# leabouffaut/DAS4Whales

Hardware: AMD Instinct MI355X
Metric: channel-samples/sec through f-k filter + matched-filter (higher is better)
Workload: dtype f32 (matched filter: 2 x f16 split operands on the matrix cores, f32 accumulate); 1 GPU; 20000 channels x 120000 samples float32 per GPU, classic f-k fan mask (fk_filter_design defaults), stages fk+mf, HF+LF fin-call templates; api=public, parallelism=independent channel blocks x1

## Files before the change

### das4whales_amd/csrc/xcorr_mm.hip

```cpp
#include <cstdlib>

#include "mm_common.h"

namespace d4w {

constexpr int kMmCH = 4096;
constexpr int kMmCHPair = 8192;
constexpr int kMmGroup = 4096;
constexpr int kMmKS = 6;
constexpr int kMmKSLong = 8;
constexpr int kMmKSMax = 16;
constexpr int kMmSection = 32 * kMmKSMax - 16;
constexpr int kMmMaxSupport = 32 * kMmKSLong - 15;
constexpr int kMmMaxSections = 16;
constexpr int kMmThreads = 256;
template <int KSM, int CH = kMmCH>
struct MmGeom {
    static constexpr int G = CH > kMmGroup ? CH / kMmGroup : 1;
    static constexpr int GL = CH / G;
    static constexpr int Halo = 32 * KSM;
    static constexpr int Stage = CH + Halo;
    static constexpr int Q = (Stage + 4 * kMmThreads - 1) / (4 * kMmThreads);
    static constexpr int LastQ = (Stage - (Q - 1) * 4 * kMmThreads) / 4;
    static constexpr int GStage = GL + Halo;
    static constexpr int Arr = G * GStage + 8;
    static constexpr int QG = GL / (4 * kMmThreads);
    static constexpr int Blk = CH / 4;
    static constexpr int Pb = G == 1 ? Blk : Blk / 4;
    static constexpr size_t lds_bytes(bool tail) {
        return (size_t)4 * Arr * sizeof(mm_half) + 8 * G * sizeof(float) + (tail ? ((size_t)2 * Pb + 2 * 16 * G) * sizeof(float) : 0);
    }
    static_assert(CH % (4 * kMmThreads) == 0 && GL % (4 * kMmThreads) == 0 && Halo <= 4 * kMmThreads, "a group is whole loads; its halo lies in one");
};

struct MmArgs {
    const float* x;
    const float* xnext;
    const double* mean;
    const float* maxabs;
    const float* taps;
    float* y0;
    float* y1;
    int nx, ns, ld_next, n_next, ltaps, len0, len1;
    float* rowmax0;
    float* rowmax1;
    int clamp;
    int shift;
    int accumulate;
    float tail0, tail1;
};

__device__ __forceinline__ int mm_tile(int wv, int ti) { return wv + 4 * ti; }

__device__ __forceinline__ float mm_wave_scan(float v) {
#ifdef D4W_EMU
    const int lane = (int)(threadIdx.x & 63);
    for (int off = 1; off < 64; off <<= 1) {
        const float n = __shfl_up(v, (unsigned)off);
        if (lane >= off) v += n;
    }
    return v;
#else
    auto dpp = [](float x, auto ctrl, auto rmask) {
        return __int_as_float(__builtin_amdgcn_update_dpp(0, __float_as_int(x), decltype(ctrl)::value, decltype(rmask)::value, 0xf, false));
    };
    v += dpp(v, std::integral_constant<int, 0x111>{}, std::integral_constant<int, 0xf>{});
    v += dpp(v, std::integral_constant<int, 0x112>{}, std::integral_constant<int, 0xf>{});
    v += dpp(v, std::integral_constant<int, 0x114>{}, std::integral_constant<int, 0xf>{});
    v += dpp(v, std::integral_constant<int, 0x118>{}, std::integral_constant<int, 0xf>{});
    v += dpp(v, std::integral_constant<int, 0x142>{}, std::integral_constant<int, 0xa>{});
    v += dpp(v, std::integral_constant<int, 0x143>{}, std::integral_constant<int, 0xc>{});
    return v;
#endif
}

template <int KS0, int KS1, int WPS, bool TAIL = false, bool WMAX = false, int CH = kMmCH>
__global__ __launch_bounds__(kMmThreads, WPS) void xcorr_mm_rows(MmArgs P) {
    constexpr int KSM = KS0 > KS1 ? KS0 : KS1;
    using GEO = MmGeom<KSM, CH>;
    constexpr int kMmHalo = GEO::Halo, kMmStage = GEO::Stage, kMmQ = GEO::Q, kMmLastQ = GEO::LastQ, kMmArr = GEO::Arr;
    constexpr int G = GEO::G, GL = GEO::GL, QG = GEO::QG, kPb = GEO::Pb;
    D4W_DYN_LDS(smem_raw);
    mm_half* lds = reinterpret_cast<mm_half*>(smem_raw);
    float* red = reinterpret_cast<float*>(lds + 4 * kMmArr);
    float* pb = red + 8 * G;
    float* wt = pb + 2 * kPb;
    const int tid = (int)threadIdx.x;
    const int lane = tid & 63, wv = mm_uniform(tid >> 6);
    const int n16 = lane & 15, g = lane >> 4;
    const int ns = P.ns;

    mm_h8 a0h[KS0], a0l[KS0];
    mm_h8 a1h[KS1 ? KS1 : 1], a1l[KS1 ? KS1 : 1];
    float osc0 = 1.f, osc1 = 1.f;
    constexpr bool kRows = TAIL;
    const int nchunk = (ns + CH - 1) / CH;
    int row_n = 0, cin_n = 0;
    size_t roff_n = 0;
    bool more_n = false;
    int left_n = 0, d_row = 0, d_cin = 0;
    if constexpr (kRows) {
        row_n = (int)blockIdx.x;
        more_n = row_n < P.nx;
    } else {
        const long long total = (long long)P.nx * nchunk;
        const int nparts = min(8, (int)gridDim.x);
        const int xcd = (int)blockIdx.x % nparts, wq = (int)blockIdx.x / nparts, nq = ((int)gridDim.x - xcd + nparts - 1) / nparts;
        const long long lo_c = total * xcd / nparts, hi_c = total * (xcd + 1) / nparts;
        const long long c_first = lo_c + wq;
        left_n = c_first < hi_c ? (int)((hi_c - c_first + nq - 1) / nq) : 0;
        row_n = (int)(c_first / nchunk);
        cin_n = (int)(c_first - (long long)row_n * nchunk);
        d_row = nq / nchunk;
        d_cin = nq - d_row * nchunk;
        more_n = left_n > 0;
    }
    roff_n = (size_t)row_n * ns;
    const size_t d_off = (size_t)(kRows ? (int)gridDim.x : d_row) * ns;
    auto advance = [&]() {
        if constexpr (kRows) {
            if (++cin_n == nchunk) { cin_n = 0; row_n += (int)gridDim.x; roff_n += d_off; }
            more_n = row_n < P.nx;
        } else {
            cin_n += d_cin; row_n += d_row; roff_n += d_off;
            if (cin_n >= nchunk) { cin_n -= nchunk; ++row_n; roff_n += (size_t)ns; }
            more_n = --left_n > 0;
        }
    };
    {
        float* tl = reinterpret_cast<float*>(smem_raw);
        constexpr int TLP = 16 + kMmHalo;
        for (int i = tid; i < 2 * TLP; i += kMmThreads) {
            const int t = i / TLP, u = i - t * TLP - 15;
            const int L = t ? P.len1 : P.len0;
            float tv = (u >= 0 && u < L && (t == 0 || KS1 > 0)) ? P.taps[(size_t)t * P.ltaps + u] : 0.f;
            if constexpr (TAIL) {
                if (u < L && (t == 0 || KS1 > 0)) tv += t ? P.tail1 : P.tail0;
            }
            tl[i] = tv;
        }
        __syncthreads();
        auto build = [&](const float* tp, int L, auto& ah, auto& al, auto ks, float& osc) {
            constexpr int KS = decltype(ks)::value;
            float m = 0.f;
            for (int i = lane; i < TLP; i += 64) m = fmaxf(m, fabsf(tp[i]));
            for (int o = 32; o > 0; o >>= 1) m = fmaxf(m, __shfl_xor(m, o));
            float up, down;
            mm_pow2_scale(m, up, down);
            osc = up;
            (void)L;
            static_for<KS>([&](auto kq) {
                constexpr int kk = decltype(kq)::value;
                static_for<8>([&](auto jq) {
                    constexpr int j = decltype(jq)::value;
                    const float v = tp[15 + 32 * kk + 8 * g + j - n16] * down;
                    mm_half hi, lo;
                    mm_split(v, hi, lo);
                    mm_set(ah[kk], j, hi);
                    mm_set(al[kk], j, lo);
                });
            });
        };
        build(tl, P.len0, a0h, a0l, std::integral_constant<int, KS0>{}, osc0);
        if constexpr (KS1 > 0) build(tl + TLP, P.len1, a1h, a1l, std::integral_constant<int, KS1>{}, osc1);
        __syncthreads();
    }

    float4 pre[kMmQ];
    Mean2 mu_n{0.f, 0.f};
    float g_n = 1.f;
    bool heavy_n = false;
    bool tail_n = false;
    int c0_n = 0;

    auto issue = [&]() {
        c0_n = cin_n * CH;
        if (!kRows || cin_n == 0) {
            mu_n = mean2_load(P.mean, row_n);
            g_n = 1.f;
            if (P.maxabs) {
                const float a = P.maxabs[row_n];
                g_n = (a > 0.f) ? 1.0f / a : 0.f;
                heavy_n = fabsf(mu_n.hi) > 0.9921875f * a;
            }
        }
        const int s0 = c0_n + P.shift;
        tail_n = s0 + kMmStage > ns;
        const float* xr = P.x + roff_n;
        const bool al = (reinterpret_cast<uintptr_t>(xr + s0) & 15) == 0;
        if (al && s0 + kMmStage <= ns) {
            const float4* p = reinterpret_cast<const float4*>(xr + s0) + tid;
            static_for<kMmQ>([&](auto qq) {
                constexpr int q = decltype(qq)::value;
                if (q < kMmQ - 1 || tid < kMmLastQ) pre[q] = mm_load4_stream(p + q * kMmThreads);
            });
        } else {
            if (al && (ns & 3) == 0) {
                static_for<kMmQ>([&](auto qq) {
                    constexpr int q = decltype(qq)::value;
                    if (q < kMmQ - 1 || tid < kMmLastQ) {
                        const int i = s0 + 4 * (tid + q * kMmThreads);
                        const float4 v = *reinterpret_cast<const float4*>(xr + min(i, ns - 4));
                        pre[q] = (i < ns) ? v : make_float4(mu_n.hi, mu_n.hi, mu_n.hi, mu_n.hi);
                    }
                });
            } else {
                static_for<kMmQ>([&](auto qq) {
                    constexpr int q = decltype(qq)::value;
                    if (q < kMmQ - 1 || tid < kMmLastQ) {
                        const int i = s0 + 4 * (tid + q * kMmThreads);
                        const float a0 = xr[min(i, ns - 1)], a1 = xr[min(i + 1, ns - 1)], a2 = xr[min(i + 2, ns - 1)], a3 = xr[min(i + 3, ns - 1)];
                        pre[q] = make_float4(i < ns ? a0 : mu_n.hi, i + 1 < ns ? a1 : mu_n.hi, i + 2 < ns ? a2 : mu_n.hi, i + 3 < ns ? a3 : mu_n.hi);
                    }
                });
            }
            if (P.xnext && P.n_next > 0 && s0 + kMmStage > ns) {
                const float* xn = P.xnext + (size_t)row_n * P.ld_next;
                const int n_next = P.n_next;
                static_for<kMmQ>([&](auto qq) {
                    constexpr int q = decltype(qq)::value;
                    if (q < kMmQ - 1 || tid < kMmLastQ) {
                        const int d = s0 + 4 * (tid + q * kMmThreads) - ns;
                        const float b0 = xn[min(max(d, 0), n_next - 1)], b1 = xn[min(max(d + 1, 0), n_next - 1)];
                        const float b2 = xn[min(max(d + 2, 0), n_next - 1)], b3 = xn[min(max(d + 3, 0), n_next - 1)];
                        if (d >= 0 && d < n_next) pre[q].x = b0;
                        if (d + 1 >= 0 && d + 1 < n_next) pre[q].y = b1;
                        if (d + 2 >= 0 && d + 2 < n_next) pre[q].z = b2;
                        if (d + 3 >= 0 && d + 3 < n_next) pre[q].w = b3;
                    }
                });
            }
        }
    };

    if (more_n) issue();
    int buf = 0;
    float pst_hi = 0.f, pst_lo = 0.f;
    for (bool more = more_n; more; more = more_n) {
        const int row = row_n, c0 = c0_n, cin = cin_n;
        const size_t roff = roff_n;
        const Mean2 mu = mu_n;
        const bool tail = tail_n;
        const int n_valid = ns + ((P.xnext && P.n_next > 0) ? P.n_next : 0) - c0 - P.shift;
        const float gout = g_n;
        const bool own_scale = !P.maxabs || heavy_n;
        float gsc[G], osx[G];
        static_for<G>([&](auto gg) { gsc[decltype(gg)::value] = g_n; osx[decltype(gg)::value] = 1.f; });
        mm_half* bh = lds + (size_t)buf * 2 * kMmArr;
        mm_half* bl = bh + kMmArr;
        advance();
        if (TAIL && cin == 0) { pst_hi = 0.f; pst_lo = 0.f; }
        if (own_scale) {
            float m[G];
            static_for<G>([&](auto gg) { m[decltype(gg)::value] = 0.f; });
            static_for<kMmQ>([&](auto qq) {
                constexpr int q = decltype(qq)::value, gq = q / QG < G ? q / QG : G - 1;
                if (q < kMmQ - 1 || tid < kMmLastQ) {
                    const float4 v = pre[q];
                    const int at = 4 * (tid + q * kMmThreads);
                    float d0 = demean(v.x, mu), d1 = demean(v.y, mu), d2 = demean(v.z, mu), d3 = demean(v.w, mu);
                    if (tail) {
                        if (at >= n_valid) d0 = 0.f;
                        if (at + 1 >= n_valid) d1 = 0.f;
                        if (at + 2 >= n_valid) d2 = 0.f;
                        if (at + 3 >= n_valid) d3 = 0.f;
                    }
                    m[gq] = fmaxf(fmaxf(m[gq], fmaxf(fabsf(d0), fabsf(d1))), fmaxf(fabsf(d2), fabsf(d3)));
                    if constexpr (q >= QG && q < G * QG && q % QG == 0) {
                        if (tid < kMmHalo / 4) m[gq - 1] = fmaxf(fmaxf(m[gq - 1], fmaxf(fabsf(d0), fabsf(d1))), fmaxf(fabsf(d2), fabsf(d3)));
                    }
                }
            });
            static_for<G>([&](auto gg) {
                constexpr int gi = decltype(gg)::value;
                for (int o = 32; o > 0; o >>= 1) m[gi] = fmaxf(m[gi], __shfl_xor(m[gi], o));
                if (lane == 0) red[wv + 4 * (gi + G * buf)] = m[gi];
            });
            lds_barrier();
            static_for<G>([&](auto gg) {
                constexpr int gi = decltype(gg)::value;
                const float* r4 = red + 4 * (gi + G * buf);
                float up, down;
                mm_pow2_scale(fmaxf(fmaxf(r4[0], r4[1]), fmaxf(r4[2], r4[3])), up, down);
                osx[gi] = mm_uniform(up);
                gsc[gi] = mm_uniform(down);
            });
        }
        auto scaled = [&](const float4 v, int at, auto gg, float (&s)[4]) {
            constexpr int gi = decltype(gg)::value;
            const float mlg = -mu.lo * gsc[gi];
            s[0] = fmaf(v.x - mu.hi, gsc[gi], mlg); s[1] = fmaf(v.y - mu.hi, gsc[gi], mlg); s[2] = fmaf(v.z - mu.hi, gsc[gi], mlg); s[3] = fmaf(v.w - mu.hi, gsc[gi], mlg);
            if (P.clamp && !own_scale) static_for<4>([&](auto ee) { constexpr int e = decltype(ee)::value; s[e] = mm_clamp_half(s[e]); });
            if (tail) {
                static_for<4>([&](auto ee) { constexpr int e = decltype(ee)::value; if (at + e >= n_valid) s[e] = 0.f; });
            }
        };
        static_for<kMmQ>([&](auto qq) {
            constexpr int q = decltype(qq)::value, gq = q / QG < G ? q / QG : G - 1;
            float s[4] = {0.f, 0.f, 0.f, 0.f};
            const bool mine = q < kMmQ - 1 || tid < kMmLastQ;
            const int at = 4 * (tid + q * kMmThreads);
#ifdef D4W_MM_V_NOCONV
            if (mine && pre[q].x == 1.2345e30f) {
#else
            if (mine) {
#endif
                scaled(pre[q], at, std::integral_constant<int, gq>{}, s);
                mm_split_put4(s, bh + (at + gq * kMmHalo), bl + (at + gq * kMmHalo));
                if constexpr (q >= QG && q < G * QG && q % QG == 0) {
                    if (tid < kMmHalo / 4) {
                        float h4[4];
                        scaled(pre[q], at, std::integral_constant<int, gq - 1>{}, h4);
                        mm_split_put4(h4, bh + (at + (gq - 1) * kMmHalo), bl + (at + (gq - 1) * kMmHalo));
                    }
                }
            }
            if constexpr (TAIL && q < G * QG) {
                const float t4 = (s[0] + s[1]) + (s[2] + s[3]);
                const float inc = mm_wave_scan(t4);
                if constexpr (G == 1) pb[buf * kPb + kMmThreads * q + tid] = inc - t4;
                else if ((lane & 3) == 0) pb[buf * kPb + (kMmThreads / 4) * q + (tid >> 2)] = inc - t4;
                if (lane == 63) wt[buf * 16 * G + 4 * q + wv] = inc;
            }
        });
        if (more_n) issue();
        lds_barrier();
        float* ya = P.y0 + roff;
        float* yb = KS1 ? P.y1 + roff : nullptr;
        const bool valign = ((reinterpret_cast<uintptr_t>(ya + c0) & 15) == 0) && (!KS1 || (reinterpret_cast<uintptr_t>(yb + c0) & 15) == 0);
        float oxs[G], o0[G], o1[G];
        static_for<G>([&](auto gg) {
            constexpr int gi = decltype(gg)::value;
            oxs[gi] = (own_scale && P.maxabs) ? osx[gi] * gout : osx[gi];
            o0[gi] = osc0 * oxs[gi];
            o1[gi] = osc1 * oxs[gi];
        });
        float segoff[G], pstg[G];
        static_for<G>([&](auto gg) { segoff[decltype(gg)::value] = 0.f; pstg[decltype(gg)::value] = 0.f; });
        constexpr int NTW = CH / 256 / 4, NST = NTW * KSM, PF = 2;
        constexpr int TG = GL / 256;
        auto frag = [&](const mm_half* arr, int ti, int kk) -> mm_h8 {
            const int T = mm_tile(wv, ti);
            const int gr = 32 * T + 2 * n16 + g + 4 * kk;
            return *reinterpret_cast<const mm_h8*>(arr + (8 * gr + (4 * ti / TG) * kMmHalo));
        };
        mm_h8 fh[PF + 1], fl[PF + 1];
        static_for<PF>([&](auto ss) {
            constexpr int s_ = decltype(ss)::value;
            fh[s_] = frag(bh, s_ / KSM, s_ % KSM);
            fl[s_] = frag(bl, s_ / KSM, s_ % KSM);
        });
        mm_f4 c0h = mm_zero(), c0l = mm_zero(), c1h = mm_zero(), c1l = mm_zero();
        float vmax0 = -INFINITY, vmax1 = -INFINITY;
        float vsum = 0.f;
        static_for<NST>([&](auto ss) {
            constexpr int s_ = decltype(ss)::value, ti = s_ / KSM, kk = s_ % KSM;
            if constexpr (s_ + PF < NST) {
                fh[(s_ + PF) % (PF + 1)] = frag(bh, (s_ + PF) / KSM, (s_ + PF) % KSM);
                fl[(s_ + PF) % (PF + 1)] = frag(bl, (s_ + PF) / KSM, (s_ + PF) % KSM);
            }
            mm_sched_fence();
            const mm_h8 xh = fh[s_ % (PF + 1)], xl = fl[s_ % (PF + 1)];
#ifndef D4W_MM_V_NOMFMA
            if constexpr (kk < KS0) {
                c0h = mm_mfma(a0h[kk], xh, c0h);
                c0l = mm_mfma(a0h[kk], xl, c0l);
            }
            if constexpr (kk < KS1) {
                c1h = mm_mfma(a1h[kk], xh, c1h);
                c1l = mm_mfma(a1h[kk], xl, c1l);
            }
            if constexpr (kk < KS0) c0l = mm_mfma(a0l[kk], xh, c0l);
            if constexpr (kk < KS1) c1l = mm_mfma(a1l[kk], xh, c1l);
#else
            c0h[0] += (float)xh[0]; c0l[0] += (float)xl[0];
#endif
            mm_sched_fence();
            if constexpr (kk == KSM - 1) {
                constexpr int tg = 4 * ti / TG;
                const int T = mm_tile(wv, ti);
                const int kl = 256 * T + 16 * n16 + 4 * g;
                const int k = c0 + kl;
                if constexpr (ti == 0) {
                    if constexpr (TAIL) {
                        static_for<G>([&](auto gg) {
                            constexpr int gi = decltype(gg)::value;
                            const float w = lane < 16 ? wt[buf * 16 * G + 16 * gi + lane] : 0.f;
                            const float inc = mm_wave_scan(w);
                            segoff[gi] = inc - w;
                            pstg[gi] = pst_hi;
#ifdef D4W_EMU
                            const float own = __shfl(inc, 15);
#else
                            const float own = __builtin_bit_cast(float, __builtin_amdgcn_readlane(__builtin_bit_cast(int, inc), 15));
#endif
                            const double pd = ((double)pst_hi + (double)pst_lo) + (double)(own * oxs[gi]);
                            const float ph = (float)pd, pl2 = (float)(pd - (double)ph);
#ifdef D4W_EMU
                            pst_hi = ph; pst_lo = pl2;
#else
                            pst_hi = __builtin_bit_cast(float, __builtin_amdgcn_readfirstlane(__builtin_bit_cast(int, ph)));
                            pst_lo = __builtin_bit_cast(float, __builtin_amdgcn_readfirstlane(__builtin_bit_cast(int, pl2)));
#endif
                        });
                    }
                }
                float r0[4], r1[4];
                float a0 = 0.f, a1 = 0.f;
                if constexpr (TAIL) {
#ifdef D4W_EMU
                    const float so = __shfl(segoff[tg], T - tg * TG);
#else
                    const float so = __builtin_bit_cast(float, __builtin_amdgcn_readlane(__builtin_bit_cast(int, segoff[tg]), T - tg * TG));
#endif
                    const int pi = G == 1 ? kMmThreads * (T >> 2) + 64 * (T & 3) + 4 * n16 : (kMmThreads / 4) * (T >> 2) + 16 * (T & 3) + n16;
                    const float pbk = fmaf(so + pb[buf * kPb + pi], oxs[tg], pstg[tg]);
                    a0 = P.tail0 * pbk;
                    a1 = P.tail1 * pbk;
                }
                static_for<4>([&](auto rr) {
                    constexpr int r = decltype(rr)::value;
                    r0[r] = fmaf(fmaf(mm_get(c0l, r), kMmLoInv, mm_get(c0h, r)), o0[tg], a0);
                    if constexpr (KS1 > 0) r1[r] = fmaf(fmaf(mm_get(c1l, r), kMmLoInv, mm_get(c1h, r)), o1[tg], a1);
                });
                c0h = mm_zero(); c0l = mm_zero(); c1h = mm_zero(); c1l = mm_zero();
#ifdef D4W_MM_V_NOSTORE
                if (r0[0] != 1.2345e30f) { }
                else
#endif
                if (valign && k + 3 < ns) {
                    if (KS1 == 0 && P.accumulate) {
                        const float4 o = mm_load4_stream(reinterpret_cast<const float4*>(ya + k));
                        r0[0] += o.x; r0[1] += o.y; r0[2] += o.z; r0[3] += o.w;
                    }
                    mm_store4(ya + k, r0[0], r0[1], r0[2], r0[3]);
                    if constexpr (KS1 > 0) mm_store4(yb + k, r1[0], r1[1], r1[2], r1[3]);
                    if (WMAX) {
                        vmax0 = fmaxf(vmax0, fmaxf(fmaxf(r0[0], r0[1]), fmaxf(r0[2], r0[3])));
                        vsum += (r0[0] + r0[1]) + (r0[2] + r0[3]);
                        if constexpr (KS1 > 0) {
                            vmax1 = fmaxf(vmax1, fmaxf(fmaxf(r1[0], r1[1]), fmaxf(r1[2], r1[3])));
                            vsum += (r1[0] + r1[1]) + (r1[2] + r1[3]);
                        }
                    }
                } else {
                    for (int r = 0; r < 4; ++r)
                        if (k + r < ns) {
                            const float v0 = (KS1 == 0 && P.accumulate) ? ya[k + r] + r0[r] : r0[r];
                            ya[k + r] = v0;
                            if constexpr (KS1 > 0) yb[k + r] = r1[r];
                            if (WMAX) {
                                vmax0 = fmaxf(vmax0, v0);
                                vsum += v0;
                                if constexpr (KS1 > 0) { vmax1 = fmaxf(vmax1, r1[r]); vsum += r1[r]; }
                            }
                        }
                }
            }
        });
        if (WMAX) {
            for (int o = 32; o > 0; o >>= 1) {
                vmax0 = fmaxf(vmax0, __shfl_xor(vmax0, o));
                if constexpr (KS1 > 0) vmax1 = fmaxf(vmax1, __shfl_xor(vmax1, o));
            }
            const bool bad = __any(vsum != vsum);
            if (lane == 0) {
                mm_atomic_fmax(P.rowmax0 + row, bad ? __uint_as_float(0x7FC00000u) : vmax0);
                if constexpr (KS1 > 0) mm_atomic_fmax(P.rowmax1 + row, bad ? __uint_as_float(0x7FC00000u) : vmax1);
            }
        }
        buf ^= 1;
    }
}

}

using namespace d4w;


constexpr int mm_wps(int ks0, int ks1, bool tail, bool wmax) { return (ks1 == 0 && ks0 <= kMmKS && !(tail && wmax)) ? 3 : 2; }

template <int KS0, int KS1, bool TAIL, bool WMAX, int CH>
static int mm_launch_as(const MmArgs& Q, int grid, void* stream) {
    constexpr size_t lds = MmGeom<(KS0 > KS1 ? KS0 : KS1), CH>::lds_bytes(TAIL);
    void (*kern)(MmArgs) = xcorr_mm_rows<KS0, KS1, mm_wps(KS0, KS1, TAIL, WMAX), TAIL, WMAX, CH>;
    if (lds > 64 * 1024) D4W_HIP(hipFuncSetAttribute((const void*)kern, hipFuncAttributeMaxDynamicSharedMemorySize, (int)lds));
    D4W_LAUNCH(kern, dim3(grid), dim3(kMmThreads), lds, stream, Q);
    return D4W_OK;
}

template <int KS0, int KS1, bool TAIL, int CH = kMmCH>
static int mm_launch(const MmArgs& Q, int grid, void* stream) {
    return Q.rowmax0 ? mm_launch_as<KS0, KS1, TAIL, true, CH>(Q, grid, stream) : mm_launch_as<KS0, KS1, TAIL, false, CH>(Q, grid, stream);
}

template <bool TAIL>
static int mm_one_section(const MmArgs& Q, int grid, void* stream) {
    const int ks = ceil_div(Q.len0 + 15, 32);
    if (ks <= kMmKS) return mm_launch<kMmKS, 0, TAIL>(Q, grid, stream);
    if (ks <= kMmKSLong) return mm_launch<kMmKSLong, 0, TAIL>(Q, grid, stream);
    if (ks <= 12) return mm_launch<12, 0, TAIL>(Q, grid, stream);
    return mm_launch<kMmKSMax, 0, TAIL>(Q, grid, stream);
}

template <bool TAIL>
static int mm_pair(const MmArgs& P, int grid, void* stream) {
    if (ceil_div(P.len0 + 15, 32) <= 5) return mm_launch<5, kMmKS, TAIL, kMmCHPair>(P, grid, stream);
    return mm_launch<kMmKS, kMmKS, TAIL, kMmCHPair>(P, grid, stream);
}

static int mm_one_template(MmArgs Q, const float* taps, int len, bool tails, float tail, float* y, float* rowmax, int grid, void* stream) {
    const int nsec = (len <= 32 * kMmKSMax - 15) ? 1 : ceil_div(len, kMmSection);
    const int per = (nsec == 1) ? len : 16 * ceil_div(ceil_div(len, nsec), 16);
    Q.y0 = y;
    Q.y1 = nullptr;
    Q.rowmax1 = nullptr;
    Q.tail0 = tail;
    Q.tail1 = 0.f;
    for (int j = 0; j < nsec; ++j) {
        const int first = j * per;
        Q.taps = taps + first;
        Q.len0 = Q.len1 = std::min(per, len - first);
        Q.shift = first;
        Q.accumulate = j > 0;
        Q.rowmax0 = (j == nsec - 1) ? rowmax : nullptr;
        const int rc = tails ? mm_one_section<true>(Q, grid, stream) : mm_one_section<false>(Q, grid, stream);
        if (rc != D4W_OK) return rc;
    }
    return D4W_OK;
}

extern "C" {

int d4w_xcorr_mm_max_support(void) { return kMmSection * kMmMaxSections; }

int d4w_xcorr_mm_f32(const float* x, int nx, int ns, const float* xnext, int ld_next, int n_next, const double* mean,
                     const float* maxabs, const float* taps, int ntpl, int ltaps, int len0, int len1, float* y0, float* y1,
                     void* stream) {
    return d4w_xcorr_mm_rowmax_f32(x, nx, ns, xnext, ld_next, n_next, mean, maxabs, taps, ntpl, ltaps, len0, len1, y0, y1, nullptr,
                                   nullptr, stream);
}

int d4w_xcorr_mm_rowmax_f32(const float* x, int nx, int ns, const float* xnext, int ld_next, int n_next, const double* mean,
                            const float* maxabs, const float* taps, int ntpl, int ltaps, int len0, int len1, float* y0, float* y1,
                            float* rowmax0, float* rowmax1, void* stream) {
    return d4w_xcorr_mm_tail_f32(x, nx, ns, xnext, ld_next, n_next, mean, maxabs, taps, ntpl, ltaps, len0, len1, 0.0, 0.0, y0, y1,
                                 rowmax0, rowmax1, stream);
}

int d4w_xcorr_mm_tail_max_support(void) { return 32 * kMmKSMax - 15; }

int d4w_xcorr_mm_tail_f32(const float* x, int nx, int ns, const float* xnext, int ld_next, int n_next, const double* mean,
                          const float* maxabs, const float* taps, int ntpl, int ltaps, int len0, int len1, double tail0, double tail1,
                          float* y0, float* y1, float* rowmax0, float* rowmax1, void* stream) {
    if (!x || !y0 || !taps || nx < 1 || ns < 1) return fail(D4W_EINVAL, "bad argument");
    if (ntpl == 2 && ((rowmax0 == nullptr) != (rowmax1 == nullptr))) return fail(D4W_EINVAL, "rowmax0 and rowmax1 go together");
    if (ntpl < 1 || ntpl > 2 || (ntpl == 2 && !y1)) return fail(D4W_EINVAL, "ntpl = %d (1 or 2 templates per call)", ntpl);
    if (xnext && (n_next < 0 || ld_next < n_next)) return fail(D4W_EINVAL, "a continuation needs 0 <= n_next <= ld_next");
    if (ntpl == 1) { len1 = len0; tail1 = 0.0; }
    if (len0 < 1 || len1 < 1 || len0 > ltaps || len1 > ltaps || std::max(len0, len1) > d4w_xcorr_mm_max_support())
        return fail(D4W_EINVAL, "template supports (%d, %d) must lie in 1..min(ltaps = %d, %d)", len0, len1, ltaps, d4w_xcorr_mm_max_support());
    const bool tails = tail0 != 0.0 || tail1 != 0.0;
    if (tails) {
        if (!mean || !maxabs) return fail(D4W_EINVAL, "the zero-padded template's tail needs the rows' statistics (mean, maxabs)");
        if (std::max(len0, len1) > d4w_xcorr_mm_tail_max_support())
            return fail(D4W_EINVAL, "with a tail the supports (%d, %d) must be <= %d", len0, len1, d4w_xcorr_mm_tail_max_support());
    }
    MmArgs P;
    P.x = x; P.xnext = xnext; P.mean = mean; P.maxabs = maxabs; P.taps = taps; P.y0 = y0; P.y1 = y1;
    P.nx = nx; P.ns = ns; P.ld_next = ld_next; P.n_next = xnext ? n_next : 0; P.ltaps = ltaps; P.len0 = len0; P.len1 = len1;
    P.shift = 0; P.accumulate = 0;
    static const int env_clamp = [] { const char* v = getenv("D4W_MM_CLAMP"); return v ? atoi(v) : 0; }();
    P.clamp = (xnext != nullptr && n_next > 0) || env_clamp;
    P.rowmax0 = rowmax0; P.rowmax1 = (ntpl == 2) ? rowmax1 : nullptr;
    P.tail0 = (float)tail0; P.tail1 = (float)tail1;
    if (rowmax0) {
        D4W_HIP(hipMemsetD32Async((hipDeviceptr_t)rowmax0, (int)0xFF800000u, (size_t)nx, (hipStream_t)stream));
        if (ntpl == 2) D4W_HIP(hipMemsetD32Async((hipDeviceptr_t)rowmax1, (int)0xFF800000u, (size_t)nx, (hipStream_t)stream));
    }
    static const int env_wgs = [] { const char* v = getenv("D4W_MM_WGS"); const int n = v ? atoi(v) : 0; return n < 0 ? 0 : (n > 8 ? 8 : n); }();
    const int ks0 = ceil_div(len0 + 15, 32), ks1 = ceil_div(len1 + 15, 32);
    const bool fused = ntpl == 2 && std::max(ks0, ks1) <= kMmKS;
    const int nchunk = ceil_div(ns, fused ? kMmCHPair : kMmCH);
    const int per_cu = env_wgs ? env_wgs : ((ntpl == 1 && ks0 <= kMmKS) ? 3 : 2);
    const long long units = tails ? (long long)nx : (long long)nx * nchunk;
    const int grid = (int)std::min<long long>(units, (long long)mm_num_cus() * per_cu);
    if (fused) return tails ? mm_pair<true>(P, grid, stream) : mm_pair<false>(P, grid, stream);
    int rc = mm_one_template(P, taps, len0, tails, P.tail0, y0, rowmax0, grid, stream);
    if (rc == D4W_OK && ntpl == 2) rc = mm_one_template(P, taps + ltaps, len1, tails, P.tail1, y1, rowmax1, grid, stream);
    return rc;
}

}
```

Before: 119.4 billion channel-samples/s.

## Add lean specialized chunk path for paired-template matched filter

Turns the per-chunk loop body into a lambda that is instantiated twice. A LEAN variant, used for paired templates when inputs are aligned, unclamped, non-accumulating and neither heavy nor at the tail, drops the own-scale reduction, clamp, tail masking and alignment checks. It also raises wave priority around the staging phase, and the tailed pair kernel now uses a smaller 4096 chunk. The cost is more template instantiations and code size, and the unchanged general path remains for the other cases.

```diff
diff --git a/das4whales_amd/csrc/xcorr_mm.hip b/das4whales_amd/csrc/xcorr_mm.hip
--- a/das4whales_amd/csrc/xcorr_mm.hip
+++ b/das4whales_amd/csrc/xcorr_mm.hip
@@ -6,6 +6,7 @@
 
 constexpr int kMmCH = 4096;
 constexpr int kMmCHPair = 8192;
+constexpr int kMmCHPairTail = 4096;
 constexpr int kMmGroup = 4096;
 constexpr int kMmKS = 6;
 constexpr int kMmKSLong = 8;
@@ -51,6 +52,13 @@
 };
 
 __device__ __forceinline__ int mm_tile(int wv, int ti) { return wv + 4 * ti; }
+
+template <int V>
+__device__ __forceinline__ void mm_wave_priority() {
+#ifndef D4W_EMU
+    __builtin_amdgcn_s_setprio(V);
+#endif
+}
 
 __device__ __forceinline__ float mm_wave_scan(float v) {
 #ifdef D4W_EMU
@@ -172,6 +180,10 @@
     bool heavy_n = false;
     bool tail_n = false;
     int c0_n = 0;
+    constexpr bool kLean = KS1 > 0;
+    const bool lean_launch = kLean && P.maxabs && !P.clamp && !P.accumulate && ((ns | P.shift) & 3) == 0 &&
+                             ((reinterpret_cast<uintptr_t>(P.x) | reinterpret_cast<uintptr_t>(P.y0) | reinterpret_cast<uintptr_t>(P.y1)) & 15) == 0;
+    bool lean_n = false;
 
     auto issue = [&]() {
         c0_n = cin_n * CH;
@@ -186,6 +198,7 @@
         }
         const int s0 = c0_n + P.shift;
         tail_n = s0 + kMmStage > ns;
+        lean_n = lean_launch && !heavy_n && !tail_n;
         const float* xr = P.x + roff_n;
         const bool al = (reinterpret_cast<uintptr_t>(xr + s0) & 15) == 0;
         if (al && s0 + kMmStage <= ns) {
@@ -236,20 +249,22 @@
     if (more_n) issue();
     int buf = 0;
     float pst_hi = 0.f, pst_lo = 0.f;
-    for (bool more = more_n; more; more = more_n) {
+    auto chunk = [&](auto lean_c) {
+        constexpr bool LEAN = decltype(lean_c)::value;
         const int row = row_n, c0 = c0_n, cin = cin_n;
         const size_t roff = roff_n;
         const Mean2 mu = mu_n;
-        const bool tail = tail_n;
+        const bool tail = LEAN ? false : tail_n;
         const int n_valid = ns + ((P.xnext && P.n_next > 0) ? P.n_next : 0) - c0 - P.shift;
         const float gout = g_n;
-        const bool own_scale = !P.maxabs || heavy_n;
+        const bool own_scale = LEAN ? false : (!P.maxabs || heavy_n);
         float gsc[G], osx[G];
         static_for<G>([&](auto gg) { gsc[decltype(gg)::value] = g_n; osx[decltype(gg)::value] = 1.f; });
         mm_half* bh = lds + (size_t)buf * 2 * kMmArr;
         mm_half* bl = bh + kMmArr;
         advance();
         if (TAIL && cin == 0) { pst_hi = 0.f; pst_lo = 0.f; }
+        if constexpr (LEAN) mm_wave_priority<1>();
         if (own_scale) {
             float m[G];
             static_for<G>([&](auto gg) { m[decltype(gg)::value] = 0.f; });
@@ -290,7 +305,7 @@
             constexpr int gi = decltype(gg)::value;
             const float mlg = -mu.lo * gsc[gi];
             s[0] = fmaf(v.x - mu.hi, gsc[gi], mlg); s[1] = fmaf(v.y - mu.hi, gsc[gi], mlg); s[2] = fmaf(v.z - mu.hi, gsc[gi], mlg); s[3] = fmaf(v.w - mu.hi, gsc[gi], mlg);
-            if (P.clamp && !own_scale) static_for<4>([&](auto ee) { constexpr int e = decltype(ee)::value; s[e] = mm_clamp_half(s[e]); });
+            if (!LEAN && P.clamp && !own_scale) static_for<4>([&](auto ee) { constexpr int e = decltype(ee)::value; s[e] = mm_clamp_half(s[e]); });
             if (tail) {
                 static_for<4>([&](auto ee) { constexpr int e = decltype(ee)::value; if (at + e >= n_valid) s[e] = 0.f; });
             }
@@ -300,11 +315,7 @@
             float s[4] = {0.f, 0.f, 0.f, 0.f};
             const bool mine = q < kMmQ - 1 || tid < kMmLastQ;
             const int at = 4 * (tid + q * kMmThreads);
-#ifdef D4W_MM_V_NOCONV
-            if (mine && pre[q].x == 1.2345e30f) {
-#else
             if (mine) {
-#endif
                 scaled(pre[q], at, std::integral_constant<int, gq>{}, s);
                 mm_split_put4(s, bh + (at + gq * kMmHalo), bl + (at + gq * kMmHalo));
                 if constexpr (q >= QG && q < G * QG && q % QG == 0) {
@@ -324,10 +335,11 @@
             }
         });
         if (more_n) issue();
+        if constexpr (LEAN) mm_wave_priority<0>();
         lds_barrier();
         float* ya = P.y0 + roff;
         float* yb = KS1 ? P.y1 + roff : nullptr;
-        const bool valign = ((reinterpret_cast<uintptr_t>(ya + c0) & 15) == 0) && (!KS1 || (reinterpret_cast<uintptr_t>(yb + c0) & 15) == 0);
+        const bool valign = LEAN || (((reinterpret_cast<uintptr_t>(ya + c0) & 15) == 0) && (!KS1 || (reinterpret_cast<uintptr_t>(yb + c0) & 15) == 0));
         float oxs[G], o0[G], o1[G];
         static_for<G>([&](auto gg) {
             constexpr int gi = decltype(gg)::value;
@@ -353,6 +365,84 @@
         mm_f4 c0h = mm_zero(), c0l = mm_zero(), c1h = mm_zero(), c1l = mm_zero();
         float vmax0 = -INFINITY, vmax1 = -INFINITY;
         float vsum = 0.f;
+        auto finish = [&](auto tt) {
+            constexpr int ti = decltype(tt)::value;
+            constexpr int tg = 4 * ti / TG;
+            const int T = mm_tile(wv, ti);
+            const int kl = 256 * T + 16 * n16 + 4 * g;
+            const int k = c0 + kl;
+            if constexpr (ti == 0) {
+                if constexpr (TAIL) {
+                    static_for<G>([&](auto gg) {
+                        constexpr int gi = decltype(gg)::value;
+                        const float w = lane < 16 ? wt[buf * 16 * G + 16 * gi + lane] : 0.f;
+                        const float inc = mm_wave_scan(w);
+                        segoff[gi] = inc - w;
+                        pstg[gi] = pst_hi;
+#ifdef D4W_EMU
+                        const float own = __shfl(inc, 15);
+#else
+                        const float own = __builtin_bit_cast(float, __builtin_amdgcn_readlane(__builtin_bit_cast(int, inc), 15));
+#endif
+                        const double pd = ((double)pst_hi + (double)pst_lo) + (double)(own * oxs[gi]);
+                        const float ph = (float)pd, pl2 = (float)(pd - (double)ph);
+#ifdef D4W_EMU
+                        pst_hi = ph; pst_lo = pl2;
+#else
+                        pst_hi = __builtin_bit_cast(float, __builtin_amdgcn_readfirstlane(__builtin_bit_cast(int, ph)));
+                        pst_lo = __builtin_bit_cast(float, __builtin_amdgcn_readfirstlane(__builtin_bit_cast(int, pl2)));
+#endif
+                    });
+                }
+            }
+            float r0[4], r1[4];
+            float a0 = 0.f, a1 = 0.f;
+            if constexpr (TAIL) {
+#ifdef D4W_EMU
+                const float so = __shfl(segoff[tg], T - tg * TG);
+#else
+                const float so = __builtin_bit_cast(float, __builtin_amdgcn_readlane(__builtin_bit_cast(int, segoff[tg]), T - tg * TG));
+#endif
+                const int pi = G == 1 ? kMmThreads * (T >> 2) + 64 * (T & 3) + 4 * n16 : (kMmThreads / 4) * (T >> 2) + 16 * (T & 3) + n16;
+                const float pbk = fmaf(so + pb[buf * kPb + pi], oxs[tg], pstg[tg]);
+                a0 = P.tail0 * pbk;
+                a1 = P.tail1 * pbk;
+            }
+            static_for<4>([&](auto rr) {
+                constexpr int r = decltype(rr)::value;
+                r0[r] = fmaf(fmaf(mm_get(c0l, r), kMmLoInv, mm_get(c0h, r)), o0[tg], a0);
+                if constexpr (KS1 > 0) r1[r] = fmaf(fmaf(mm_get(c1l, r), kMmLoInv, mm_get(c1h, r)), o1[tg], a1);
+            });
+            c0h = mm_zero(); c0l = mm_zero(); c1h = mm_zero(); c1l = mm_zero();
+            if (LEAN || (valign && k + 3 < ns)) {
+                if (KS1 == 0 && P.accumulate) {
+                    const float4 o = mm_load4_stream(reinterpret_cast<const float4*>(ya + k));
+                    r0[0] += o.x; r0[1] += o.y; r0[2] += o.z; r0[3] += o.w;
+                }
+                mm_store4(ya + k, r0[0], r0[1], r0[2], r0[3]);
+                if constexpr (KS1 > 0) mm_store4(yb + k, r1[0], r1[1], r1[2], r1[3]);
+                if (WMAX) {
+                    vmax0 = fmaxf(vmax0, fmaxf(fmaxf(r0[0], r0[1]), fmaxf(r0[2], r0[3])));
+                    vsum += (r0[0] + r0[1]) + (r0[2] + r0[3]);
+                    if constexpr (KS1 > 0) {
+                        vmax1 = fmaxf(vmax1, fmaxf(fmaxf(r1[0], r1[1]), fmaxf(r1[2], r1[3])));
+                        vsum += (r1[0] + r1[1]) + (r1[2] + r1[3]);
+                    }
+                }
+            } else {
+                for (int r = 0; r < 4; ++r)
+                    if (k + r < ns) {
+                        const float v0 = (KS1 == 0 && P.accumulate) ? ya[k + r] + r0[r] : r0[r];
+                        ya[k + r] = v0;
+                        if constexpr (KS1 > 0) yb[k + r] = r1[r];
+                        if (WMAX) {
+                            vmax0 = fmaxf(vmax0, v0);
+                            vsum += v0;
+                            if constexpr (KS1 > 0) { vmax1 = fmaxf(vmax1, r1[r]); vsum += r1[r]; }
+                        }
+                    }
+            }
+        };
         static_for<NST>([&](auto ss) {
             constexpr int s_ = decltype(ss)::value, ti = s_ / KSM, kk = s_ % KSM;
             if constexpr (s_ + PF < NST) {
@@ -361,7 +451,6 @@
             }
             mm_sched_fence();
             const mm_h8 xh = fh[s_ % (PF + 1)], xl = fl[s_ % (PF + 1)];
-#ifndef D4W_MM_V_NOMFMA
             if constexpr (kk < KS0) {
                 c0h = mm_mfma(a0h[kk], xh, c0h);
                 c0l = mm_mfma(a0h[kk], xl, c0l);
@@ -372,91 +461,8 @@
             }
             if constexpr (kk < KS0) c0l = mm_mfma(a0l[kk], xh, c0l);
             if constexpr (kk < KS1) c1l = mm_mfma(a1l[kk], xh, c1l);
-#else
-            c0h[0] += (float)xh[0]; c0l[0] += (float)xl[0];
-#endif
             mm_sched_fence();
-            if constexpr (kk == KSM - 1) {
-                constexpr int tg = 4 * ti / TG;
-                const int T = mm_tile(wv, ti);
-                const int kl = 256 * T + 16 * n16 + 4 * g;
-                const int k = c0 + kl;
-                if constexpr (ti == 0) {
-                    if constexpr (TAIL) {
-                        static_for<G>([&](auto gg) {
-                            constexpr int gi = decltype(gg)::value;
-                            const float w = lane < 16 ? wt[buf * 16 * G + 16 * gi + lane] : 0.f;
-                            const float inc = mm_wave_scan(w);
-                            segoff[gi] = inc - w;
-                            pstg[gi] = pst_hi;
-#ifdef D4W_EMU
-                            const float own = __shfl(inc, 15);
-#else
-                            const float own = __builtin_bit_cast(float, __builtin_amdgcn_readlane(__builtin_bit_cast(int, inc), 15));
-#endif
-                            const double pd = ((double)pst_hi + (double)pst_lo) + (double)(own * oxs[gi]);
-                            const float ph = (float)pd, pl2 = (float)(pd - (double)ph);
-#ifdef D4W_EMU
-                            pst_hi = ph; pst_lo = pl2;
-#else
-                            pst_hi = __builtin_bit_cast(float, __builtin_amdgcn_readfirstlane(__builtin_bit_cast(int, ph)));
-                            pst_lo = __builtin_bit_cast(float, __builtin_amdgcn_readfirstlane(__builtin_bit_cast(int, pl2)));
-#endif
-                        });
-                    }
-                }
-                float r0[4], r1[4];
-                float a0 = 0.f, a1 = 0.f;
-                if constexpr (TAIL) {
-#ifdef D4W_EMU
-                    const float so = __shfl(segoff[tg], T - tg * TG);
-#else
-                    const float so = __builtin_bit_cast(float, __builtin_amdgcn_readlane(__builtin_bit_cast(int, segoff[tg]), T - tg * TG));
-#endif
-                    const int pi = G == 1 ? kMmThreads * (T >> 2) + 64 * (T & 3) + 4 * n16 : (kMmThreads / 4) * (T >> 2) + 16 * (T & 3) + n16;
-                    const float pbk = fmaf(so + pb[buf * kPb + pi], oxs[tg], pstg[tg]);
-                    a0 = P.tail0 * pbk;
-                    a1 = P.tail1 * pbk;
-                }
-                static_for<4>([&](auto rr) {
-                    constexpr int r = decltype(rr)::value;
-                    r0[r] = fmaf(fmaf(mm_get(c0l, r), kMmLoInv, mm_get(c0h, r)), o0[tg], a0);
-                    if constexpr (KS1 > 0) r1[r] = fmaf(fmaf(mm_get(c1l, r), kMmLoInv, mm_get(c1h, r)), o1[tg], a1);
-                });
-                c0h = mm_zero(); c0l = mm_zero(); c1h = mm_zero(); c1l = mm_zero();
-#ifdef D4W_MM_V_NOSTORE
-                if (r0[0] != 1.2345e30f) { }
-                else
-#endif
-                if (valign && k + 3 < ns) {
-                    if (KS1 == 0 && P.accumulate) {
-                        const float4 o = mm_load4_stream(reinterpret_cast<const float4*>(ya + k));
-                        r0[0] += o.x; r0[1] += o.y; r0[2] += o.z; r0[3] += o.w;
-                    }
-                    mm_store4(ya + k, r0[0], r0[1], r0[2], r0[3]);
-                    if constexpr (KS1 > 0) mm_store4(yb + k, r1[0], r1[1], r1[2], r1[3]);
-                    if (WMAX) {
-                        vmax0 = fmaxf(vmax0, fmaxf(fmaxf(r0[0], r0[1]), fmaxf(r0[2], r0[3])));
-                        vsum += (r0[0] + r0[1]) + (r0[2] + r0[3]);
-                        if constexpr (KS1 > 0) {
-                            vmax1 = fmaxf(vmax1, fmaxf(fmaxf(r1[0], r1[1]), fmaxf(r1[2], r1[3])));
-                            vsum += (r1[0] + r1[1]) + (r1[2] + r1[3]);
-                        }
-                    }
-                } else {
-                    for (int r = 0; r < 4; ++r)
-                        if (k + r < ns) {
-                            const float v0 = (KS1 == 0 && P.accumulate) ? ya[k + r] + r0[r] : r0[r];
-                            ya[k + r] = v0;
-                            if constexpr (KS1 > 0) yb[k + r] = r1[r];
-                            if (WMAX) {
-                                vmax0 = fmaxf(vmax0, v0);
-                                vsum += v0;
-                                if constexpr (KS1 > 0) { vmax1 = fmaxf(vmax1, r1[r]); vsum += r1[r]; }
-                            }
-                        }
-                }
-            }
+            if constexpr (kk == KSM - 1) finish(std::integral_constant<int, ti>{});
         });
         if (WMAX) {
             for (int o = 32; o > 0; o >>= 1) {
@@ -470,6 +476,14 @@
             }
         }
         buf ^= 1;
+    };
+    if constexpr (kLean) {
+        while (more_n) {
+            while (more_n && lean_n) chunk(std::true_type{});
+            if (more_n) chunk(std::false_type{});
+        }
+    } else {
+        while (more_n) chunk(std::false_type{});
     }
 }
 
@@ -505,8 +519,9 @@
 
 template <bool TAIL>
 static int mm_pair(const MmArgs& P, int grid, void* stream) {
-    if (ceil_div(P.len0 + 15, 32) <= 5) return mm_launch<5, kMmKS, TAIL, kMmCHPair>(P, grid, stream);
-    return mm_launch<kMmKS, kMmKS, TAIL, kMmCHPair>(P, grid, stream);
+    constexpr int CH = TAIL ? kMmCHPairTail : kMmCHPair;
+    if (ceil_div(P.len0 + 15, 32) <= 5) return mm_launch<5, kMmKS, TAIL, CH>(P, grid, stream);
+    return mm_launch<kMmKS, kMmKS, TAIL, CH>(P, grid, stream);
 }
 
 static int mm_one_template(MmArgs Q, const float* taps, int len, bool tails, float tail, float* y, float* rowmax, int grid, void* stream) {
```

Result: faster. 121.4 billion channel-samples/s, median of 6 (+1.6%).
